# Kolkir/feature-point-cnn

Hardware: AMD Instinct MI355X
Metric: frames/sec (VGA 640x480) SuperPoint fwd+NMS+descriptors (higher is better)
Workload: dtype f32

## Files before the change

### feature-point-cnn_amd/_lib.py

```python
import ctypes
import os
import subprocess

import torch

_DIR = os.path.dirname(os.path.abspath(__file__))
LIB_PATH = os.environ.get("FPC_LIB_PATH") or os.path.join(_DIR, "lib", "libfpc.so")
CSRC = os.path.join(_DIR, "csrc")

SYMBOLS = [
    "fpc_abi_version", "fpc_build_flags", "fpc_strerror", "fpc_last_hip_error", "fpc_default_config", "fpc_create",
    "fpc_destroy", "fpc_load_weights", "fpc_packed_size", "fpc_packed_device_ptr",
    "fpc_export_packed", "fpc_import_packed", "fpc_import_packed_device", "fpc_mark_weights_loaded", "fpc_set_stream", "fpc_upload_stream",
    "fpc_get_stream", "fpc_sync", "fpc_forward", "fpc_detect", "fpc_get_points", "fpc_results",
    "fpc_get_counts", "fpc_get_keypoints", "fpc_set_timing", "fpc_get_timings", "fpc_match", "fpc_first_within",
    "fpc_detect_u8", "fpc_u8_staging", "fpc_homography_adaptation", "fpc_detect_u8_resized",
    "fpc_sample_descriptors", "fpc_plan_hash", "fpc_broadcast_weights", "fpc_read_activation",
    "fpc_pack_layout_revision", "fpc_check_guards", "fpc_stream_report", "fpc_output_range",
    "fpc_match_frames", "fpc_first_within_frames",
    "fpc_default_ransac_params", "fpc_ransac_homography", "fpc_homography_frames",
    "fpc_bank_create", "fpc_bank_destroy", "fpc_bank_get", "fpc_bank_store", "fpc_bank_store_rows", "fpc_bank_clear",
    "fpc_match_bank", "fpc_homography_bank", "fpc_bank_create_ex", "fpc_bank_format",
    "fpc_match_frames_guided", "fpc_match_bank_guided",
    "fpc_cell_order", "fpc_match_frames_guided_cells", "fpc_match_bank_guided_cells",
    "fpc_bank_topk_reserve", "fpc_match_bank_topk", "fpc_homography_bank_topk",
    "fpc_ransac_fundamental", "fpc_fundamental_frames", "fpc_fundamental_bank",
    "fpc_match_frames_guided_epipolar", "fpc_match_bank_guided_epipolar",
    "fpc_match_frames_guided_epipolar_cells", "fpc_match_bank_guided_epipolar_cells",
    "fpc_default_pose_params", "fpc_pose_fundamental", "fpc_pose_frames", "fpc_pose_bank",
]

ABI_VERSION = 4
PACK_LAYOUT_REVISION = 4

PLAN_FLAGS = {
    "no_fused_blocks": 1 << 0, "no_winograd": 1 << 1, "no_winograd_detector": 1 << 2, "no_winograd_layer_in1": 1 << 3,
    "no_xcd_order": 1 << 4, "no_fused_stem_pool": 1 << 5, "split_heads": 1 << 6, "nms_in_line": 1 << 7,
    "no_persistent_grid": 1 << 8, "layer1_tile_8x16": 1 << 9, "winograd_gen1": 1 << 10, "no_latency_tiles": 1 << 11,
    "nms_one_workgroup": 1 << 12, "no_fused_softmax": 1 << 13, "winograd_gen2": 1 << 14, "guard_zones": 1 << 15, "detector_gen1": 1 << 16, "heads_in_line": 1 << 17, "w36_one_wave": 1 << 18, "convt_phases": 1 << 19, "stem_round3": 1 << 20, "conv_round1": 1 << 21,
}


class FpcConfig(ctypes.Structure):
    _fields_ = [("device", ctypes.c_int), ("height", ctypes.c_int), ("width", ctypes.c_int),
                ("max_batch", ctypes.c_int), ("cell", ctypes.c_int), ("nms_dist", ctypes.c_int),
                ("conf_thresh", ctypes.c_float), ("border_remove", ctypes.c_int),
                ("descriptor_enabled", ctypes.c_int), ("max_keypoints", ctypes.c_int),
                ("in_channels", ctypes.c_int), ("dtype", ctypes.c_int), ("arch", ctypes.c_int),
                ("num_streams", ctypes.c_int), ("plan_flags", ctypes.c_uint), ("nms_round_launches", ctypes.c_int),
                ("min_sub_batch", ctypes.c_int)]


class FpcTensor(ctypes.Structure):
    _fields_ = [("name", ctypes.c_char_p), ("data", ctypes.c_void_p), ("ndim", ctypes.c_int),
# ... 172 lines not shown
```

### feature-point-cnn_amd/csrc/fpc_api.hip

```cpp
#include <hip/hip_runtime.h>

#include <dlfcn.h>

#include <algorithm>
#include <cmath>
#include <cstdio>
#include <cstdlib>
#include <cstring>
#include <memory>
#include <mutex>
#include <chrono>
#include <string>
#include <vector>

#include "../../include/fpc.h"
#include "block_mfma.h"
#include "block_bf16.h"
#include "convt_bf16.h"
#include "block_x3.h"
#include "stem_bf16.h"
#include "wblock_mfma.h"
#include "wblock16_mfma.h"
#include "wblock36_mfma.h"
#include "wblock36p_mfma.h"
// ... 194 lines not shown
      WK_COUNT
};

struct WKindInfo {
  const char* name;
  const char* symbol;
  int gen;
  int KC, NBT, CMID, lds_bytes;
  int NCG;
  int TH;
  int TW;
  int threads;
  const void* fn;
  void (*launch)(const WBlockArgs&, dim3, hipStream_t);
  bool dust = false;
};

#define X(name, KC, NBT, CMID)                                                                            \
  static void launchw_##name(const WBlockArgs& a, dim3 grid, hipStream_t st) {                            \
    constexpr int lds = WBlockCfg<KC, NBT, CMID>::LDS_BYTES;                                              \
    hipLaunchKernelGGL((wblock_mfma_kernel<KC, NBT, CMID>), grid, dim3(512), lds, st, a);                 \
  }
FPC_WBLOCK_KINDS(X)
#undef X
#define X(name, NCG, TH)                                                                                  \
  static void launchw_##name(const WBlockArgs& a, dim3 grid, hipStream_t st) {                            \
    constexpr int lds = W16Cfg<NCG, TH>::LDS_BYTES;                                                       \
    hipLaunchKernelGGL((wblock16_kernel<NCG, TH>), grid, dim3(512), lds, st, a);                          \
  }
FPC_W16_KINDS(X)
// ... 28 lines not shown
#undef X

static const WKindInfo g_wkinds[WK_COUNT] = {
#define X(name, KC, NBT, CMID)                                                                            \
  {#name, "wblock_mfma_kernel<" #KC ", " #NBT ", " #CMID ">", 1, KC, NBT, CMID,                           \
   WBlockCfg<KC, NBT, CMID>::LDS_BYTES, 0, 8, 16, 512, (const void*)wblock_mfma_kernel<KC, NBT, CMID>, launchw_##name},
    FPC_WBLOCK_KINDS(X)
#undef X
#define X(name, NCG, TH)                                                                                  \
  {#name, "wblock16_kernel<" #NCG ", " #TH ">", 2, 16, NCG / 2, NCG * 16,                                  \
   W16Cfg<NCG, TH>::LDS_BYTES, NCG, TH, 16, 512, (const void*)wblock16_kernel<NCG, TH>, launchw_##name},
    FPC_W16_KINDS(X)
#undef X
#define X(name, NB, TYT, TXT)                                                                             \
  {#name, "wblock36_kernel<" #NB ", " #TYT ", " #TXT ">", 3, 16, 2 * NB, 64 * NB,                          \
   W36Cfg<NB, TYT, TXT>::LDS_BYTES, 4 * NB, 4 * TYT, 4 * TXT, 256, (const void*)wblock36_kernel<NB, TYT, TXT>, launchw_##name},
    FPC_W36_KINDS(X)
#undef X
#define X(name, TYT, TXT)                                                                                 \
  {#name, "wblock36_dust_kernel<" #TYT ", " #TXT ">", 3, 16, 2, 64,                                        \
   W36Cfg<1, TYT, TXT, true>::LDS_BYTES, 4, 4 * TYT, 4 * TXT, 256, (const void*)wblock36_dust_kernel<TYT, TXT>, launchw_##name, true},
    FPC_W36D_KINDS(X)
#undef X
#define X(name, TYT, TXT)                                                                                 \
  {#name, "wblock36p_kernel<" #TYT ", " #TXT ", 3>", 3, 16, 2, 64,                                            \
   W36PCfg<TYT, TXT>::LDS_BYTES, 4, 4 * TYT, 4 * TXT, 512, (const void*)wblock36p_kernel<TYT, TXT>, launchw_##name},
    FPC_W36P_KINDS(X)
#undef X
#define X(name, TYT, TXT)                                                                                 \
  {#name, "wblock36p_dust_kernel<" #TYT ", " #TXT ", 3>", 3, 16, 2, 64,                                    \
   W36PCfg<TYT, TXT, true>::LDS_BYTES, 4, 4 * TYT, 4 * TXT, 512, (const void*)wblock36p_dust_kernel<TYT, TXT>, launchw_##name, true},
    FPC_W36PD_KINDS(X)
#undef X
};

static size_t w1_floats(const WKindInfo& k, int nchunk) {
  if (k.gen == 3) return (size_t)k.NCG * ((size_t)nchunk * 36 + (k.NCG == 8 ? W36Cfg<2, 4, 4>::WPAD : W36Cfg<1, 4, 4>::WPAD)) * 256;
  return (size_t)k.NCG * ((size_t)nchunk * 16 + W16Cfg<8>::WPAD) * 256;
}
static double wkind_mfma_flops(const WKindInfo& k, int tiles, int nchunk, int k8_1x1) {
  const double px = (double)k.TH * k.TW, n = k.NBT * 32.0;
  if (k.gen == 3) return 2.0 * tiles * n * (36.0 * (px / 16) * nchunk * k.KC + px * k8_1x1 * 8.0);
  return 2.0 * tiles * n * (16.0 * (px / 4) * nchunk * k.KC + px * k8_1x1 * 8.0);
}
static bool w36_fits(int , int H, int W, int cs_in, int cs_out) {
  return (unsigned long long)H * W * (unsigned long long)std::max(cs_in, cs_out) * sizeof(float) < (unsigned long long)W36_MARKER;
// ... 109 lines not shown
  int pH = 0, pW = 0, pC = 0;
  std::string prefix;
  int cin = 0, cout = 0;
  int grid_y = 1, grid_z = 1;
  double flops_per_frame = 0;
  double mfma_flops_per_frame = 0;
  bool fused_softmax_capable = false;
  double bytes_per_frame = 0;
  bool descriptor_branch = false;
};

struct Timing {
  hipEvent_t start, stop;
  int op;
  int frames;
};

}

using namespace fpc;

struct fpc_ctx {
  fpc_config cfg{};
  int H = 0, W = 0, B = 0, Hc = 0, Wc = 0;
  bool vgg = false;
  int D = 128;
  std::vector<float*> vbuf;
  size_t vconv0_off = 0;
  bool bf16 = false;
  bool split = false;
// ... 26 lines not shown
  bool logits_valid = false;
  bool nms_one_workgroup = false;
  int nms_g = 0;
  bool fuse_stem_pool = true;
  bool conv_lean = true;
  bool stem_lean = true;
  bool stem2 = false;
  bool layer1_t816 = false;
#ifdef FPC_DIAG
  unsigned long long* diag_stamps = nullptr;
  int diag_n = 0;
#endif
  bool winograd_in1 = true;
  bool winograd_det = true;
  int w36_cus = 0;
  bool w36_paired = true;
  bool winograd_det_gen3 = true;
  bool winograd = true;
  bool latency_tiles = true;
  int winograd_gen = 3;
  bool fuse_blocks = true;
  bool weights_loaded = false;
  bool plan_error = false;

  char* slab = nullptr;
  size_t slab_bytes = 0;
  bool guard_zones = false;
  std::vector<std::pair<size_t, size_t>> guards;
  float *stem_out, *x0, *h4, *x1, *x2, *h8, *x3, *cat, *dh, *dproj, *d0, *lg;
  float *h16, *y16a, *y16b, *lo_h, *lo0, *desc_map, *desc_in_nhwc;
// ... 1295 lines not shown
  c->stem2 = c->stem_lean && !c->bf16 && !c->split && !c->vgg && (c->fuse_stem_pool || c->cin == 1) && H2 % 2 == 0 && W2 % STEM_T == 0;
  return FPC_OK;
}

static uint64_t plan_hash(const fpc_ctx* c) {
  uint64_t h = 1469598103934665603ull;
  auto mix = [&](uint64_t v) {
    for (int i = 0; i < 8; ++i) {
      h ^= (v >> (8 * i)) & 0xff;
      h *= 1099511628211ull;
    }
  };
  mix(FPC_ABI_VERSION); mix(FPC_PACK_LAYOUT_REVISION); mix((uint64_t)c->cfg.dtype); mix((uint64_t)c->cfg.arch); mix((uint64_t)c->cin);
  mix((uint64_t)(c->cfg.descriptor_enabled != 0)); mix(c->blob_floats); mix(c->stem_w_off); mix(c->stem_b_off);
  mix(c->vconv0_off);
  for (size_t i = 0; i < c->ops.size(); ++i) {
    const Op& op = c->ops[i];
    mix((uint64_t)op.type); mix((uint64_t)op.kind); mix((uint64_t)op.bkind); mix((uint64_t)op.wkind); mix((uint64_t)op.fkind);
    mix((uint64_t)(op.phase + 1)); mix((uint64_t)op.n0);
    for (char ch : op.prefix) mix((uint64_t)(unsigned char)ch);
    const fpc_ctx::ConvW& cw = c->convw[i];
    for (int z = 0; z < 4; ++z) mix(cw.w_off[z]);
    mix(cw.b_off); mix(cw.b2_off);
  }
  return h;
}

static void fill_blob_header(const fpc_ctx* c, uint32_t* h) {
  memset(h, 0, BLOB_HEADER_FLOATS * sizeof(uint32_t));
  const uint64_t ph = plan_hash(c);
// ... 500 lines not shown
struct Sub {
  int f0, n;
  bool small = false;
  bool fuse_softmax = false;
  hipStream_t st;
  hipStream_t side = nullptr;
  hipEvent_t ev_enc = nullptr, ev_det = nullptr;
};

struct LaunchTimer {
  fpc_ctx* c;
  int op;
  hipStream_t st;
  int frames;
  hipEvent_t s{}, e{};
  LaunchTimer(fpc_ctx* c_, int op_, hipStream_t st_, int frames_) : c(c_), op(op_), st(st_), frames(frames_) {
    if (c->timing) {
      s = next_event(c);
      e = next_event(c);
      hipEventRecord(s, st);
    }
  }
  ~LaunchTimer() {
    if (c->timing) {
      hipEventRecord(e, st);
      c->timings.push_back({s, e, op, frames});
    }
  }
};

static int op_index(const fpc_ctx* c, OpType t) {
  for (size_t i = 0; i < c->ops.size(); ++i)
    if (c->ops[i].type == t) return (int)i;
  return -1;
}

static void run_network(fpc_ctx* c, const float* frames, const Sub& sb0, int which, hipStream_t st) {
  Sub sb = sb0;
  sb.st = st;
  const int H = c->H, W = c->W, n = sb.n, f0 = sb.f0;
  for (size_t i = 0; i < c->ops.size(); ++i) {
// ... 88 lines not shown
            a.stamps = c->diag_stamps;
            c->diag_n = a.tiles_x * a.tiles_y * n;
          }
#endif
        a.total = a.tiles_x * a.tiles_y * n;
        a.xcd_order = c->xcd_order ? 1 : 0;
        {
          const unsigned long long xb = (unsigned long long)(f0 + n) * a.H * a.W * a.csx * sizeof(float);
          a.x_bytes = xb > 0xfffffff0ull ? 0xfffffff0u : (unsigned)xb;
        }
        int grid = (c->persist_min_tiles > 0 && a.total >= c->persist_min_tiles * c->num_cus) ? c->num_cus : a.total;
        if (g_wkinds[op.wkind].gen == 3) {
          const int fpl = w36_frames_per_launch(a.H, a.W, a.csx, a.cso);
          const float* x0 = a.x;
          float* o0 = a.out;
          for (int g0 = 0; g0 < n; g0 += fpl) {
            const int gn = std::min(fpl, n - g0);
            a.frame0 = 0;
            a.x = x0 + (size_t)(f0 + g0) * a.H * a.W * a.csx;
            a.out = o0 + (size_t)(f0 + g0) * a.H * a.W * a.cso;
            a.total = a.tiles_x * a.tiles_y * gn;
            a.x_bytes = (unsigned)((unsigned long long)gn * a.H * a.W * a.csx * sizeof(float));
            const int cus_cap = c->w36_cus > 0 ? std::min(c->num_cus, c->w36_cus) : c->num_cus;
            const int cus8 = std::max(1, cus_cap / 8 / std::max(1, op.grid_y)), per_xcd = (a.total + 7) / 8;
            const int rounds = (per_xcd + cus8 - 1) / cus8;
            const int grid3 = 8 * std::min(cus8, (per_xcd + rounds - 1) / rounds);
            g_wkinds[op.wkind].launch(a, dim3(std::min(a.total, grid3), op.grid_y), sb.st);
          }
          break;
        }
        g_wkinds[op.wkind].launch(a, dim3(std::min(a.total, grid), op.grid_y), sb.st);
        break;
      }
      case OP_BLOCK: {
        LaunchTimer t(c, (int)i, sb.st, n);
        BlockArgs a = op.bargs;
        a.frame0 = f0;
#ifdef FPC_DIAG
        a.stamps = nullptr;
        if (const char* e = getenv("FPC_STAMP_OP"))
          if (op.name.find(e) != std::string::npos) {
            if (!c->diag_stamps) hipHostMalloc((void**)&c->diag_stamps, (size_t)65536 * 8 * sizeof(unsigned long long));
            memset(c->diag_stamps, 0, (size_t)65536 * 8 * sizeof(unsigned long long));
// ... 373 lines not shown
  const auto create_t0 = std::chrono::steady_clock::now();
  std::unique_lock<std::mutex> queue_lock(qmap::state().mu);
  const int probe_rounds0 = qmap::state().dev[cfg->device].rounds;
  c->stream = qmap::acquire(cfg->device, c.get(), SLOT_MAIN, true, qprobe, true);
  if (!c->stream) { qmap::release_owner(c.get()); g_hip_err = "hipStreamCreateWithFlags"; return FPC_E_HIP; }
  c->own_stream = true;
  {
    int nsub = cfg->num_streams > 0 ? std::min(8, cfg->num_streams) : (c->split ? 3 : 2);
    const unsigned pf = cfg->plan_flags;
    c->fuse_blocks = !(pf & FPC_PLAN_NO_FUSED_BLOCKS);
    c->guard_zones = (pf & FPC_PLAN_GUARD_ZONES) != 0;
    if (const char* e = getenv("FPC_GUARD_ZONES")) c->guard_zones = atoi(e) != 0;
    c->winograd_det_gen3 = !(pf & FPC_PLAN_DETECTOR_GEN1);
    c->w36_paired = !(pf & FPC_PLAN_W36_ONE_WAVE);
    if (const char* e = getenv("FPC_W36_PAIRED")) c->w36_paired = atoi(e) != 0;
    if (const char* e = getenv("FPC_W36_CUS")) c->w36_cus = std::max(0, atoi(e));
    if (const char* e = getenv("FPC_WINOGRAD_DET_GEN")) c->winograd_det_gen3 = atoi(e) >= 3;
    c->winograd = !(pf & FPC_PLAN_NO_WINOGRAD);
    c->winograd_det = !(pf & FPC_PLAN_NO_WINOGRAD_DETECTOR);
    c->winograd_in1 = !(pf & FPC_PLAN_NO_WINOGRAD_LAYER_IN1);
    c->xcd_order = !(pf & FPC_PLAN_NO_XCD_ORDER);
    c->fuse_stem_pool = !(pf & FPC_PLAN_NO_FUSED_STEM_POOL);
    c->stem_lean = !(pf & FPC_PLAN_STEM_ROUND3);
    c->conv_lean = !(pf & FPC_PLAN_CONV_ROUND1);
    if (const char* e = getenv("FPC_CONV_LEAN")) c->conv_lean = atoi(e) != 0;
    if (const char* e = getenv("FPC_STEM_LEAN")) c->stem_lean = atoi(e) != 0;
    c->split_heads = (pf & FPC_PLAN_SPLIT_HEADS) != 0;
    if (pf & FPC_PLAN_NO_PERSISTENT_GRID) c->persist_min_tiles = 0;
    c->layer1_t816 = (pf & FPC_PLAN_LAYER1_TILE_8x16) != 0;
    c->winograd_gen = (pf & FPC_PLAN_WINOGRAD_GEN1) ? 1 : (pf & FPC_PLAN_WINOGRAD_GEN2) ? 2 : 3;
// ... 1466 lines not shown
          case OP_CONV: k = op->lean ? lean_kind(op->kind)->symbol : g_kinds[op->kind].symbol; break;
          case OP_BLOCK: k = g_bkinds[op->bkind].symbol; break;
          case OP_WBLOCK: k = g_wkinds[op->wkind].symbol; break;
          case OP_BF16: k = g_fkinds[op->fkind].symbol; break;
          case OP_SOFTMAX: k = "softmax_d2s_kernel"; break;
          case OP_NMS: k = c->nms_one_workgroup ? "nms_rounds_kernel+nms_sort_kernel" : "nms_rounds_kernel+nms_finish_kernel+nms_chunk_sort_kernel+nms_merge_kernel"; break;
          case OP_DESC: k = "descriptor16_kernel"; break;
          case OP_VCONV0: k = "vgg_conv0_kernel"; break;
          case OP_POOL2: k = "maxpool2_kernel"; break;
          case OP_L2NORM: k = "l2norm256_kernel"; break;
        }
      kernels[i] = k;
    }
    if (ms) ms[i] = v;
    if (flops) flops[i] = op ? op->flops_per_frame * t.frames : 0.0;
    if (mfma_flops) mfma_flops[i] = op ? op->mfma_flops_per_frame * t.frames : 0.0;
    if (bytes) bytes[i] = op ? op->bytes_per_frame * t.frames : 0.0;
  }
  return n;
}

}
```

### feature-point-cnn_amd/csrc/wblock36_mfma.h

```cpp
#pragma once
#include <type_traits>
#include <utility>

#include "wblock16_mfma.h"

namespace fpc {

template <int... I, class F>
__device__ __forceinline__ void fpc_static_for_impl(std::integer_sequence<int, I...>, F&& f) {
  (f(std::integral_constant<int, I>{}), ...);
}
template <int N, class F>
__device__ __forceinline__ void fpc_static_for(F&& f) {
  fpc_static_for_impl(std::make_integer_sequence<int, N>{}, f);
}

struct W36Dust {
  static constexpr int W2ROW = 0, W2COL = 64, WPCOL = 144, B1 = 400, B2 = 401, UIN64 = 404, UIN = 448, UOUT = 448 + 4 * 36 * 16;
  static constexpr int floats(int nchunk) { return UOUT + nchunk * 36 * 16; }
};

template <int NB_, int TYT_, int TXT_, bool DUST_ = false>
struct W36Cfg {
  static constexpr int NB = NB_, TYT = TYT_, TXT = TXT_;
// ... 188 lines not shown
  auto t_burst = [&]() {
#pragma unroll
    for (int jj = 0; jj < 3; ++jj) bt6(tp[0][jj], tp[1][jj], tp[2][jj], tp[3][jj], tp[4][jj], tp[5][jj]);
#pragma unroll
    for (int ii = 0; ii < 3; ++ii)
#pragma unroll
      for (int jj = 0; jj < 3; ++jj) {
        const f32x2 ra = tp[2 * ii][jj], rb = tp[2 * ii + 1][jj];
        tp[2 * ii][jj] = __builtin_shufflevector(ra, rb, 0, 2);
        tp[2 * ii + 1][jj] = __builtin_shufflevector(ra, rb, 1, 3);
      }
#pragma unroll
    for (int ii = 0; ii < 3; ++ii) bt6(tp[2 * ii][0], tp[2 * ii + 1][0], tp[2 * ii][1], tp[2 * ii + 1][1], tp[2 * ii][2], tp[2 * ii + 1][2]);
  };
  auto t_write = [&](int wr, int i, int j) { lds[wr + (i * 6 + j) * 256] = tp[2 * (i >> 1) + (j & 1)][j >> 1][i & 1]; };
  auto transform_all = [&](int hoff, int voff) {
#pragma unroll
    for (int i = 0; i < 6; ++i)
#pragma unroll
      for (int j = 0; j < 6; ++j) t_read(trd + hoff, i, j);
    t_burst();
#pragma unroll
    for (int i = 0; i < 6; ++i)
#pragma unroll
      for (int j = 0; j < 6; ++j) t_write(twr + voff, i, j);
  };

  const int aoff4 = (lane & 15) * 4 + ((lane >> 4) ^ (2 * ((lane & 15) >> 3)));
  const unsigned gstride = ((unsigned)nchunk * 36u + (unsigned)C::WPAD) * 1024u;
  const __amdgpu_buffer_rsrc_t wrsrc = __builtin_amdgcn_make_buffer_rsrc(const_cast<float4*>(w1h), 0, (int)(4u * (unsigned)NB * gstride), 0x00020000);
  const unsigned wlane = (unsigned)(wave * NB) * gstride + lane16;
  const int gs_s = __builtin_amdgcn_readfirstlane((int)gstride);
  struct BF { f32x4 v[2][NB]; };
  auto ldb = [&](int s) {
    BF r;
// ... 13 lines not shown
  if constexpr (DUST) {
    d_va = wave * 64 + lane;
    d_ua = wave * 64 + 16 * ((lane & 3) ^ (2 * (lane >> 5)));
    for (int i = tid; i < 448 / 4; i += NT) lds4[C::D_HEAD / 4 + i] = reinterpret_cast<const f32x4*>(a.dust)[i];
    for (int i = tid; i < 2304 / 4; i += NT) lds4[C::D_UIN / 4 + i] = reinterpret_cast<const f32x4*>(a.dust + W36Dust::UIN)[i];
  }

  TilePos pos_cur = tile_pos(wg_first);
  int base_cur = halo_base(pos_cur);
  halo_tile(pos_cur);
  load_halo64(base_cur);
  load_halo(base_cur, C::OFF_H0);
  load_halo(base_cur + 64, C::OFF_H1);
  asm volatile("s_waitcnt vmcnt(%0)" ::"n"(HIT) : "memory");
  FPC_LDS_BARRIER();
  transform_all(C::OFF_H0, C::OFF_V0);
  FPC_LDS_BARRIER();

  constexpr int C4 = N / 4, EIT = HPX * C4 / NT, PPI = NT / C4;
  constexpr int CPR = TW / PPI;
  const __amdgpu_buffer_rsrc_t orsrc = __builtin_amdgcn_make_buffer_rsrc(a.out + blockIdx.y * N, 0, W36_MARKER, 0x00020000);

  const int g2s = __builtin_amdgcn_readfirstlane(((a.k8_h + a.k8_x) / 2 + C::WPAD2) * 64);
  const __amdgpu_buffer_rsrc_t w2rsrc = __builtin_amdgcn_make_buffer_rsrc(const_cast<float4*>(a.w2), 0, a.conv_only ? 0 : 4 * NB * g2s * 16, 0x00020000);
  const unsigned w2lane = (unsigned)(wave * NB * g2s) * 16u + lane16;

  const int wg_stamp = wg_first + 2 * wg_step < wg_end ? wg_first + 2 * wg_step : wg_first;
  for (int wg = wg_first; wg < wg_end; wg += wg_step) {
    const int b = pos_cur.b, ty = pos_cur.ty, tx = pos_cur.tx;
    const TilePos pos_next = tile_pos(wg + wg_step);
// ... 16 lines not shown
    if constexpr (DUST) {
      float zf = 0.f;
      asm volatile("" : "+v"(zf));
#pragma unroll
      for (int i = 0; i < 9; ++i) dacc[i] = zf;
    }

    auto chunk_body = [&](auto PAR, const int c) {
      constexpr int par = decltype(PAR)::value;
      constexpr int VB_OFF = par ? C::OFF_V1 : C::OFF_V0, VN_OFF = par ? C::OFF_V0 : C::OFF_V1;
      constexpr int HS_OFF = par ? C::OFF_H1 : C::OFF_H0;
      constexpr int HN_OFF = par ? C::OFF_H0 : C::OFF_H1;
      const int c3 = c + 2;
      const bool nxt = c3 >= nchunk;
      const int l_base = (nxt ? base_next : base_cur) + (nxt ? c3 - nchunk : c3) * 64;
      int ao = aoff4 + VB_OFF / 4, trd_c = trd + HN_OFF, twr_c = twr + VN_OFF;
      asm volatile("" : "+v"(ao), "+v"(trd_c), "+v"(twr_c));
      [[maybe_unused]] int dva = d_va + VB_OFF / 4;
      [[maybe_unused]] f32x4 dv[3];
      if constexpr (DUST) asm volatile("" : "+v"(dva));
      constexpr int AQ = 2;
      f32x4 ac[2][AQ];
#pragma unroll
      for (int q = 0; q < AQ; ++q) ac[0][q] = lds4[ao + q * 64];
#ifdef FPC_DIAG_STEPS
      unsigned long long tq[11] = {0, 0, 0, 0, 0, 0, 0, 0, 0, 0, 0};
#define FPC_TQ(i) asm volatile("s_memtime %0" : "=s"(tq[i]));
#else
#define FPC_TQ(i)
#endif
      fpc_static_for<STEPS>([&](auto S) __attribute__((always_inline)) {
        constexpr int s = decltype(S)::value;
        if constexpr (s % 2 == 0) { FPC_TQ(s / 2) }
        bq[(s + RING - 1) % RING] = ldb(c * STEPS + s + RING - 1);
        if (s + 1 < STEPS) {
#pragma unroll
          for (int q = 0; q < AQ; ++q) ac[(s + 1) & 1][q] = lds4[ao + ((s + 1) * AQ + q) * 64];
        }
        constexpr int SPS = 36 / STEPS;
#pragma unroll
        for (int u = 0; u < SPS; ++u) {
          const int slot = s * SPS + u;
          if (slot == 1) {
            if (c3 == nchunk) halo_tile(pos_next);
            load_halo(l_base, HS_OFF);
          } else if (slot >= 2 && slot < 14) {
#pragma unroll
            for (int k = 0; k < 3; ++k) { const int e = (slot - 2) * 3 + k; t_read(trd_c, e / 6, e % 6); }
          } else if (slot == 14) {
            t_burst();
          } else if (slot >= 15 && slot < 33) {
#pragma unroll
            for (int k = 0; k < 2; ++k) { const int e = (slot - 15) * 2 + k; t_write(twr_c, e / 6, e % 6); }
          }
          if constexpr (DUST) {
            auto dread = [&](int i0) {
#pragma unroll
              for (int k = 0; k < 3; ++k) dv[k] = lds4[dva + (i0 + k) * 256];
            };
            auto dfma = [&](int i0) {
#pragma unroll
              for (int k = 0; k < 3; ++k)
#pragma unroll
// ... 28 lines not shown
        }
        __builtin_amdgcn_sched_barrier(0);
      });
      FPC_TQ(9)
      asm volatile("s_waitcnt vmcnt(%0)" ::"n"(2 * NB * (RING - 1)) : "memory");
      FPC_LDS_BARRIER();
      FPC_TQ(10)
#ifdef FPC_DIAG_STEPS
      if (a.stamps && wg == wg_stamp && c == 2 && (threadIdx.x & 63) == 0) {
        asm volatile("s_waitcnt lgkmcnt(0)" ::: "memory");
        unsigned long long* q = a.stamps + 1024 * 8 + ((size_t)blockIdx.x * 4 + (threadIdx.x >> 6)) * 16;
        for (int i = 0; i < 11; ++i) q[i] = tq[i];
      }
#endif
    };
    __builtin_amdgcn_s_waitcnt(0x0F70);
    {
      int c = 0;
      do {
        chunk_body(std::integral_constant<int, 0>{}, c);
        chunk_body(std::integral_constant<int, 1>{}, c + 1);
        c += 2;
      } while (c < nchunk);
    }
    if (wg == wg_stamp) { FPC_STAMP(1) }
    asm volatile("s_nop 15\n\ts_nop 7" ::: "memory");

    if constexpr (DUST) {
      int tid_d = tid;
      asm volatile("" : "+v"(tid_d));
// ... 430 lines not shown
```

### feature-point-cnn_amd/csrc/wblock36p_mfma.h

```cpp
#pragma once
#include "wblock36_mfma.h"

namespace fpc {

template <int TYT_, int TXT_, bool DUST_ = false>
struct W36PCfg {
  static constexpr int TYT = TYT_, TXT = TXT_;
  static constexpr bool DUST = DUST_;
  static_assert(TYT * TXT == 16 && (TYT == 4 || TYT == 2), "16 Winograd tiles per workgroup tile: 4 x 4 or 2 x 8");
  static constexpr int NT = 512, NTH = 256, NPOS = 36, KC = 16, N = 64;
  static constexpr int TH = 4 * TYT, TW = 4 * TXT, HH = TH + 2, HW = TW + 2, NHALO = HH * HW;
  static constexpr int HROW = 20;
  static constexpr int HIT = (NHALO * 5 + NTH - 1) / NTH;
  static constexpr int HALO_FLOATS = HIT * NTH * 4;
  static constexpr int V_FLOATS = NPOS * 16 * 16;
  static constexpr int OFF_V0 = 0, OFF_H1 = V_FLOATS, OFF_H0 = OFF_H1 + HALO_FLOATS, OFF_V1 = OFF_H0 + HALO_FLOATS;
  static constexpr int RH = N + 8;
  static constexpr int PX = TH * TW;
  static constexpr int T_FLOATS = PX * RH;
  static constexpr int BASE_FLOATS = (OFF_V1 + V_FLOATS) > (OFF_H0 + T_FLOATS) ? (OFF_V1 + V_FLOATS) : (OFF_H0 + T_FLOATS);
  static constexpr int HIT64 = (NHALO + NTH - 1) / NTH;
  static constexpr int D_HEAD = BASE_FLOATS, D_COL = D_HEAD + 64, D_UIN = D_HEAD + 448, D_V64 = D_UIN + 2304, D_M64 = D_V64 + 576, D_H64 = D_M64 + 576;
  static constexpr int LDS_FLOATS = DUST ? D_H64 + HIT64 * NTH * 4 : BASE_FLOATS;
  static constexpr int LDS_BYTES = LDS_FLOATS * 4;
// ... 144 lines not shown
  auto t_burst = [&]() {
#pragma unroll
    for (int jj = 0; jj < 3; ++jj) bt6(tp[0][jj], tp[1][jj], tp[2][jj], tp[3][jj], tp[4][jj], tp[5][jj]);
#pragma unroll
    for (int ii = 0; ii < 3; ++ii)
#pragma unroll
      for (int jj = 0; jj < 3; ++jj) {
        const f32x2 ra = tp[2 * ii][jj], rb = tp[2 * ii + 1][jj];
        tp[2 * ii][jj] = __builtin_shufflevector(ra, rb, 0, 2);
        tp[2 * ii + 1][jj] = __builtin_shufflevector(ra, rb, 1, 3);
      }
#pragma unroll
    for (int ii = 0; ii < 3; ++ii) bt6(tp[2 * ii][0], tp[2 * ii + 1][0], tp[2 * ii][1], tp[2 * ii + 1][1], tp[2 * ii][2], tp[2 * ii + 1][2]);
  };
  auto t_write = [&](int wr, int i, int j) { lds[wr + (i * 6 + j) * 256] = tp[2 * (i >> 1) + (j & 1)][j >> 1][i & 1]; };

  const int aoff4 = (lane & 15) * 4 + ((lane >> 4) ^ (2 * ((lane & 15) >> 3))) + hs * 18 * 64;
  const unsigned gstride = ((unsigned)nchunk * 36u + (unsigned)C::WPAD) * 1024u;
  const __amdgpu_buffer_rsrc_t wrsrc = __builtin_amdgcn_make_buffer_rsrc(const_cast<float4*>(w1h), 0, (int)(4u * gstride), 0x00020000);
  const unsigned wlane = (unsigned)grp * gstride + (unsigned)hs * (18u * 1024u) + lane16;
  struct BF { f32x4 v[2]; };
  auto ldb = [&](int cc, int s) {
    BF r;
#pragma unroll
    for (int q = 0; q < 2; ++q)
      r.v[q] = __builtin_bit_cast(f32x4, __builtin_amdgcn_raw_buffer_load_b128(wrsrc, (int)wlane, cc * (36 * 1024) + (2 * s + q) * 1024, 0));
    return r;
  };

  [[maybe_unused]] int d_va = 0, d_ua = 0;
// ... 7 lines not shown
    for (int i = tid; i < 448 / 4; i += C::NT) lds4[C::D_HEAD / 4 + i] = reinterpret_cast<const f32x4*>(a.dust)[i];
    for (int i = tid; i < 2304 / 4; i += C::NT) lds4[C::D_UIN / 4 + i] = reinterpret_cast<const f32x4*>(a.dust + W36Dust::UIN)[i];
  }

  TilePos pos_cur = tile_pos(wg_first);
  int base_cur = halo_base(pos_cur);
  if (hs == 1) {
    halo_tile(pos_cur);
    load_halo64(base_cur);
    load_halo(base_cur, C::OFF_H0);
    load_halo(base_cur + 64, C::OFF_H1);
    asm volatile("s_waitcnt vmcnt(%0)" ::"n"(HIT) : "memory");
  }
  FPC_LDS_BARRIER();
  if (hs == 0) {
#pragma unroll
    for (int i = 0; i < 6; ++i)
#pragma unroll
      for (int j = 0; j < 6; ++j) t_read(trd + C::OFF_H0, i, j);
    t_burst();
#pragma unroll
    for (int i = 0; i < 6; ++i)
#pragma unroll
      for (int j = 0; j < 6; ++j) t_write(twr + C::OFF_V0, i, j);
  }
  FPC_LDS_BARRIER();

  constexpr int C4 = N / 4, EIT = PX * C4 / C::NT, PPI = C::NT / C4;
  constexpr int RPI = PPI / TW > 0 ? PPI / TW : 1;
  const __amdgpu_buffer_rsrc_t orsrc = __builtin_amdgcn_make_buffer_rsrc(a.out + blockIdx.y * N, 0, W36_MARKER, 0x00020000);
  const int g2s = __builtin_amdgcn_readfirstlane(((a.k8_h + a.k8_x) / 2 + C::WPAD2) * 64);
  const __amdgpu_buffer_rsrc_t w2rsrc = __builtin_amdgcn_make_buffer_rsrc(const_cast<float4*>(a.w2), 0, a.conv_only ? 0 : 4 * g2s * 16, 0x00020000);
  const unsigned w2lane = (unsigned)(grp * g2s) * 16u + lane16;

// ... 17 lines not shown
#pragma unroll
      for (int i = 0; i < 9; ++i) dacc[i] = zf;
    }
    BF bq[RING];
#pragma unroll
    for (int i = 0; i < RING - 1; ++i) bq[i] = ldb(0, i);

    auto chunk_body = [&](auto ROLE, auto PAR, const int c) {
      constexpr int role = decltype(ROLE)::value, par = decltype(PAR)::value;
      constexpr int VB_OFF = par ? C::OFF_V1 : C::OFF_V0, VN_OFF = par ? C::OFF_V0 : C::OFF_V1;
      constexpr int HS_OFF = par ? C::OFF_H1 : C::OFF_H0;
      constexpr int HN_OFF = par ? C::OFF_H0 : C::OFF_H1;
      const int c3 = c + 2;
      const bool nxt = c3 >= nchunk;
      const int l_base = (nxt ? base_next : base_cur) + (nxt ? c3 - nchunk : c3) * 64;
      int ao = aoff4 + VB_OFF / 4, trd_c = trd + HN_OFF, twr_c = twr + VN_OFF;
      asm volatile("" : "+v"(ao), "+v"(trd_c), "+v"(twr_c));
      [[maybe_unused]] int dva = d_va + VB_OFF / 4;
      [[maybe_unused]] f32x4 dv[3];
      if constexpr (DUST) asm volatile("" : "+v"(dva));
      f32x4 ac[2][2];
#pragma unroll
      for (int q = 0; q < 2; ++q) ac[0][q] = lds4[ao + q * 64];
      fpc_static_for<STEPS>([&](auto S) __attribute__((always_inline)) {
        constexpr int s = decltype(S)::value;
        {
          constexpr int t = s + RING - 1;
          if constexpr (t < STEPS) bq[t % RING] = ldb(c, t);
          else bq[t % RING] = ldb(c + 1, t - STEPS);
        }
        if (s + 1 < STEPS) {
#pragma unroll
// ... 23 lines not shown
#pragma unroll
                for (int k = 0; k < 3; ++k)
                  du[(i0 / 3 % 2) * 3 + k] = __builtin_bit_cast(f32x4, __builtin_amdgcn_raw_buffer_load_b128(drsrc, d_ua + (i0 + k) * 256, c * (36 * 16 * 4), 0));
              };
              if (slot == 3) dload(0);
              else if (slot == 11) dread(0);
              else if (slot == 13) { dfma(0); dload(3); }
              else if (slot == 21) dread(3);
              else if (slot == 23) { dfma(3); dload(6); }
              else if (slot == 31) dread(6);
              else if (slot == 33) dfma(6);
            }
          } else {
            if (slot >= 2 && slot < 14) {
#pragma unroll
              for (int k = 0; k < 3; ++k) { const int e = (slot - 2) * 3 + k; t_read(trd_c, e / 6, e % 6); }
            } else if (slot == 14) {
              t_burst();
            } else if (slot >= 15 && slot < 33) {
#pragma unroll
              for (int k = 0; k < 2; ++k) { const int e = (slot - 15) * 2 + k; t_write(twr_c, e / 6, e % 6); }
            }
          }
        }
        __builtin_amdgcn_sched_barrier(0);
        fpc_mfma_step<false, false>(acc[2 * s], acc[2 * s + 1], ac[s & 1][0], ac[s & 1][1], bq[s % RING].v[0], bq[s % RING].v[1]);
        __builtin_amdgcn_sched_barrier(0);
      });
      asm volatile("s_waitcnt vmcnt(%0)" ::"n"(2 * (STEPS - 1)) : "memory");
      FPC_LDS_BARRIER();
    };
    __builtin_amdgcn_s_waitcnt(0x0F70);
    if (hs == 0) {
      int c = 0;
      do {
        chunk_body(std::integral_constant<int, 0>{}, std::integral_constant<int, 0>{}, c);
        chunk_body(std::integral_constant<int, 0>{}, std::integral_constant<int, 1>{}, c + 1);
        c += 2;
      } while (c < nchunk);
    } else {
      int c = 0;
      do {
        chunk_body(std::integral_constant<int, 1>{}, std::integral_constant<int, 0>{}, c);
        chunk_body(std::integral_constant<int, 1>{}, std::integral_constant<int, 1>{}, c + 1);
        c += 2;
      } while (c < nchunk);
    }
    if (wg == wg_stamp) { FPC_STAMP(1) }
    asm volatile("s_nop 15\n\ts_nop 7" ::: "memory");

    int tid_t = tid;
    asm volatile("" : "+v"(tid_t));
    const int lane_t = tid_t & 63, n16 = lane_t & 15, kq = lane_t >> 4;
    const bool proj = a.k8_x > 0;
    if constexpr (DUST) {
      if (a.dust_in) {
        if (tid_t < 16) {
          const int rd = C::D_H64 + ((4 * (tid_t / TXT)) * HW + 4 * (tid_t % TXT)) * 4;
#pragma unroll
          for (int i = 0; i < 6; ++i)
#pragma unroll
            for (int j = 0; j < 6; ++j) tp[i][j >> 1][j & 1] = lds[rd + (i * HW + j) * 4];
          t_burst();
          const int mrow = ((tid_t & 7) >> 1) * 4 + (tid_t >> 3) * 2 + (tid_t & 1);
#pragma unroll
          for (int i = 0; i < 6; ++i)
#pragma unroll
            for (int j = 0; j < 6; ++j) lds[C::D_V64 + (i * 6 + j) * 16 + mrow] = tp[2 * (i >> 1) + (j & 1)][j >> 1][i & 1];
        }
        FPC_LDS_BARRIER();
        {
          const int va = C::D_V64 + hs * 18 * 16 + (lane_t & 15), ub = C::D_UIN + grp * 576 + hs * 18 * 16 + (lane_t & 15);
          float av[18], bv[18];
#pragma unroll
          for (int p = 0; p < 18; ++p) {
            av[p] = lds[va + p * 16];
            bv[p] = lds[ub + p * 16];
// ... 216 lines not shown
            cb[(u + 3) & 3] = ldb2(s_first + g + u + 3);
            fpc_static_for<4>([&](auto B_) __attribute__((always_inline)) {
              constexpr int blk = decltype(B_)::value;
              if (blk + 1 < 4) {
#pragma unroll
                for (int q = 0; q < 2; ++q) af[(blk + 1) & 1][q] = lds4[ar + (g + u) * 4 + ((blk + 1) * 2 + q) * 16 * (RH / 4)];
              } else {
#pragma unroll
                for (int q = 0; q < 2; ++q) af[(blk + 1) & 1][q] = lds4[ar + (g + u + 1) * 4 + q * 16 * (RH / 4)];
              }
              __builtin_amdgcn_sched_barrier(0);
              fpc_mfma_step<false, false>(acc2[2 * blk], acc2[2 * blk + 1], af[blk & 1][0], af[blk & 1][1], cb[u], cb[u]);
              __builtin_amdgcn_sched_barrier(0);
            });
          }
        }
      };
      if (proj) {
        constexpr int XIT = PX * 16 / C::NT;
        f32x4 xst[XIT];
        auto load_x = [&](int pass) {
          const int kx4 = min(16, a.k8_x * 2 - pass * 16);
          const int px0 = tid_t >> 4;
          const int xp = (((px0 / TW) * a.W + px0 % TW) * a.csx + ((tid_t & 15) < kx4 ? pass * 64 + (tid_t & 15) * 4 : 0)) * 4;
#pragma unroll
          for (int i = 0; i < XIT; ++i) {
            const int so = xbase + i * RPI * a.W * a.csx * 4;
            xst[i] = __builtin_bit_cast(f32x4, __builtin_amdgcn_raw_buffer_load_b128(xrsrc, xp + so, 0, 0));
          }
        };
// ... 116 lines not shown
```

### feature-point-cnn_amd/csrc/wblock_mfma.h

```cpp
#pragma once
#include "block_mfma.h"

namespace fpc {

struct WBlockArgs {
  const float* x;
  int csx, nchunk;
  int H, W;
  const float4* w1;
  const float* b1;
  const float4* w2;
  const float* b2;
  int k8_h, k8_x;
  float* out;
  int cso, tiles_x, tiles_y, frame0;
  int total;
  int xcd_order;
  int ysplit_floats;
  unsigned x_bytes;
  int conv_only;
  const float* dust;
  int dust_in;
#ifdef FPC_DIAG
  unsigned long long* stamps;
#endif
};

template <int KC, int NBT, int CMID_>
struct WBlockCfg {
  static constexpr int TH = 8, TW = 16, NT = 512;
  static constexpr int HW = TW + 2, HH = TH + 2;
  static constexpr int ROW4 = KC / 4 + 1;
  static constexpr int CMID = CMID_;
  static constexpr int ROWH4 = CMID / 4 + 1;
  static constexpr int HALO_BYTES = HH * HW * ROW4 * 16;
  static constexpr int V_BYTES = 16 * 32 * ROW4 * 16;
  static constexpr int M_BYTES = 16 * 32 * 36 * 4;
// ... 408 lines not shown
```

### include/fpc.h

```cpp
#ifndef FPC_H
#define FPC_H

#include <stddef.h>
#include <stdint.h>

#ifdef __cplusplus
extern "C" {
#endif

#define FPC_ABI_VERSION 4
#define FPC_PACK_LAYOUT_REVISION 4

enum {
  FPC_OK = 0,
  FPC_E_INVALID = -1,
  FPC_E_NO_DEVICE = -2,
  FPC_E_HIP = -3,
  FPC_E_NO_WEIGHTS = -4,
  FPC_E_MISSING_KEY = -5,
  FPC_E_CAPACITY = -6,
  FPC_E_NOT_CONVERGED = -7,
  FPC_E_RANGE = -8,
  FPC_E_NONFINITE = -9
};
// ... 30 lines not shown
  FPC_PLAN_NO_FUSED_STEM_POOL = 1 << 5,
  FPC_PLAN_SPLIT_HEADS = 1 << 6,
  FPC_PLAN_NMS_IN_LINE = 1 << 7,
  FPC_PLAN_NO_PERSISTENT_GRID = 1 << 8,
  FPC_PLAN_LAYER1_TILE_8x16 = 1 << 9,
  FPC_PLAN_WINOGRAD_GEN1 = 1 << 10,
  FPC_PLAN_NO_LATENCY_TILES = 1 << 11,
  FPC_PLAN_NMS_ONE_WORKGROUP = 1 << 12,
  FPC_PLAN_NO_FUSED_SOFTMAX = 1 << 13,
  FPC_PLAN_WINOGRAD_GEN2 = 1 << 14,
  FPC_PLAN_HEADS_IN_LINE = 1 << 17,
  FPC_PLAN_DETECTOR_GEN1 = 1 << 16,
  FPC_PLAN_W36_ONE_WAVE = 1 << 18,
  FPC_PLAN_STEM_ROUND3 = 1 << 20,
  FPC_PLAN_CONV_ROUND1 = 1 << 21,
  FPC_PLAN_CONVT_PHASES = 1 << 19,
  FPC_PLAN_GUARD_ZONES = 1 << 15
};

typedef struct fpc_tensor {
  const char* name;
  const float* data;
  int ndim;
  int64_t shape[4];
} fpc_tensor;

typedef struct fpc_device_results {
  const int32_t* count;
  const int32_t* n_candidates;
  const int32_t* xy;
// ... 199 lines not shown
```

Measured before the change: 12090.

## Stack frames vertically in Winograd F(4,3) kernels to avoid partial edge tiles

When the frame height is a multiple of 4 but not of 16, the Winograd block kernels now treat a group of frames as one tall image, so 16-row tiles span frame boundaries instead of each frame ending in a partly empty tile. Rows that touch a frame boundary are redirected to zero-padding in LDS, using a magic-number modulo to find the per-frame row. This cuts wasted tile work at frame edges in exchange for extra per-tile index arithmetic and added complexity. Timing accounting scales MFMA flops by the number of tiles actually walked, and a plan flag and env var can turn the behaviour off.

Result: no change. 12180 (median of 6 runs) (+0.8%).

```diff
diff --git a/feature-point-cnn_amd/_lib.py b/feature-point-cnn_amd/_lib.py
--- a/feature-point-cnn_amd/_lib.py
+++ b/feature-point-cnn_amd/_lib.py
@@ -38,6 +38,7 @@
     "no_xcd_order": 1 << 4, "no_fused_stem_pool": 1 << 5, "split_heads": 1 << 6, "nms_in_line": 1 << 7,
     "no_persistent_grid": 1 << 8, "layer1_tile_8x16": 1 << 9, "winograd_gen1": 1 << 10, "no_latency_tiles": 1 << 11,
     "nms_one_workgroup": 1 << 12, "no_fused_softmax": 1 << 13, "winograd_gen2": 1 << 14, "guard_zones": 1 << 15, "detector_gen1": 1 << 16, "heads_in_line": 1 << 17, "w36_one_wave": 1 << 18, "convt_phases": 1 << 19, "stem_round3": 1 << 20, "conv_round1": 1 << 21,
+    "w36_no_stack": 1 << 22,
 }
 
 
diff --git a/feature-point-cnn_amd/csrc/fpc_api.hip b/feature-point-cnn_amd/csrc/fpc_api.hip
--- a/feature-point-cnn_amd/csrc/fpc_api.hip
+++ b/feature-point-cnn_amd/csrc/fpc_api.hip
@@ -232,6 +232,7 @@
   const void* fn;
   void (*launch)(const WBlockArgs&, dim3, hipStream_t);
   bool dust = false;
+  bool stack = false;
 };
 
 #define X(name, KC, NBT, CMID)                                                                            \
@@ -290,7 +291,8 @@
 #undef X
 #define X(name, NB, TYT, TXT)                                                                             \
   {#name, "wblock36_kernel<" #NB ", " #TYT ", " #TXT ">", 3, 16, 2 * NB, 64 * NB,                          \
-   W36Cfg<NB, TYT, TXT>::LDS_BYTES, 4 * NB, 4 * TYT, 4 * TXT, 256, (const void*)wblock36_kernel<NB, TYT, TXT>, launchw_##name},
+   W36Cfg<NB, TYT, TXT>::LDS_BYTES, 4 * NB, 4 * TYT, 4 * TXT, 256, (const void*)wblock36_kernel<NB, TYT, TXT>, launchw_##name, \
+   false, NB == 2 && TYT == 4},
     FPC_W36_KINDS(X)
 #undef X
 #define X(name, TYT, TXT)                                                                                 \
@@ -300,12 +302,14 @@
 #undef X
 #define X(name, TYT, TXT)                                                                                 \
   {#name, "wblock36p_kernel<" #TYT ", " #TXT ", 3>", 3, 16, 2, 64,                                            \
-   W36PCfg<TYT, TXT>::LDS_BYTES, 4, 4 * TYT, 4 * TXT, 512, (const void*)wblock36p_kernel<TYT, TXT>, launchw_##name},
+   W36PCfg<TYT, TXT>::LDS_BYTES, 4, 4 * TYT, 4 * TXT, 512, (const void*)wblock36p_kernel<TYT, TXT>, launchw_##name, false, \
+   TYT == 4},
     FPC_W36P_KINDS(X)
 #undef X
 #define X(name, TYT, TXT)                                                                                 \
   {#name, "wblock36p_dust_kernel<" #TYT ", " #TXT ", 3>", 3, 16, 2, 64,                                    \
-   W36PCfg<TYT, TXT, true>::LDS_BYTES, 4, 4 * TYT, 4 * TXT, 512, (const void*)wblock36p_dust_kernel<TYT, TXT>, launchw_##name, true},
+   W36PCfg<TYT, TXT, true>::LDS_BYTES, 4, 4 * TYT, 4 * TXT, 512, (const void*)wblock36p_dust_kernel<TYT, TXT>, launchw_##name, true, \
+   TYT == 4},
     FPC_W36PD_KINDS(X)
 #undef X
 };
@@ -445,6 +449,7 @@
   hipEvent_t start, stop;
   int op;
   int frames;
+  double mfma_scale = 1.0;
 };
 
 }
@@ -501,6 +506,7 @@
   bool winograd_in1 = true;
   bool winograd_det = true;
   int w36_cus = 0;
+  bool w36_stack = true;
   bool w36_paired = true;
   bool winograd_det_gen3 = true;
   bool winograd = true;
@@ -1826,6 +1832,7 @@
   mix(FPC_ABI_VERSION); mix(FPC_PACK_LAYOUT_REVISION); mix((uint64_t)c->cfg.dtype); mix((uint64_t)c->cfg.arch); mix((uint64_t)c->cin);
   mix((uint64_t)(c->cfg.descriptor_enabled != 0)); mix(c->blob_floats); mix(c->stem_w_off); mix(c->stem_b_off);
   mix(c->vconv0_off);
+  if (!c->w36_stack) mix(0x5733364e4f53544bull);
   for (size_t i = 0; i < c->ops.size(); ++i) {
     const Op& op = c->ops[i];
     mix((uint64_t)op.type); mix((uint64_t)op.kind); mix((uint64_t)op.bkind); mix((uint64_t)op.wkind); mix((uint64_t)op.fkind);
@@ -2356,6 +2363,7 @@
   hipStream_t st;
   int frames;
   hipEvent_t s{}, e{};
+  double mfma_scale = 1.0;
   LaunchTimer(fpc_ctx* c_, int op_, hipStream_t st_, int frames_) : c(c_), op(op_), st(st_), frames(frames_) {
     if (c->timing) {
       s = next_event(c);
@@ -2366,7 +2374,7 @@
   ~LaunchTimer() {
     if (c->timing) {
       hipEventRecord(e, st);
-      c->timings.push_back({s, e, op, frames});
+      c->timings.push_back({s, e, op, frames, mfma_scale});
     }
   }
 };
@@ -2485,19 +2493,29 @@
           const int fpl = w36_frames_per_launch(a.H, a.W, a.csx, a.cso);
           const float* x0 = a.x;
           float* o0 = a.out;
+          const int H1 = a.H, tiles_y1 = a.tiles_y;
+          const bool stackable = c->w36_stack && g_wkinds[op.wkind].stack && g_wkinds[op.wkind].TH == 16 && H1 % 4 == 0 && H1 % 16 != 0;
+          long long walked = 0;
           for (int g0 = 0; g0 < n; g0 += fpl) {
             const int gn = std::min(fpl, n - g0);
+            const bool stacked = stackable && gn >= 2 && (long long)gn * H1 + 16 < 65536;
             a.frame0 = 0;
-            a.x = x0 + (size_t)(f0 + g0) * a.H * a.W * a.csx;
-            a.out = o0 + (size_t)(f0 + g0) * a.H * a.W * a.cso;
-            a.total = a.tiles_x * a.tiles_y * gn;
-            a.x_bytes = (unsigned)((unsigned long long)gn * a.H * a.W * a.csx * sizeof(float));
+            a.x = x0 + (size_t)(f0 + g0) * H1 * a.W * a.csx;
+            a.out = o0 + (size_t)(f0 + g0) * H1 * a.W * a.cso;
+            a.H = stacked ? gn * H1 : H1;
+            a.tiles_y = stacked ? (gn * H1 + 15) / 16 : tiles_y1;
+            a.stack_h = stacked ? H1 : 0;
+            a.stack_magic = stacked ? (unsigned)(0x100000000ull / (unsigned)H1) + 1u : 0u;
+            a.total = stacked ? a.tiles_x * a.tiles_y : a.tiles_x * a.tiles_y * gn;
+            a.x_bytes = (unsigned)((unsigned long long)gn * H1 * a.W * a.csx * sizeof(float));
             const int cus_cap = c->w36_cus > 0 ? std::min(c->num_cus, c->w36_cus) : c->num_cus;
             const int cus8 = std::max(1, cus_cap / 8 / std::max(1, op.grid_y)), per_xcd = (a.total + 7) / 8;
             const int rounds = (per_xcd + cus8 - 1) / cus8;
             const int grid3 = 8 * std::min(cus8, (per_xcd + rounds - 1) / rounds);
             g_wkinds[op.wkind].launch(a, dim3(std::min(a.total, grid3), op.grid_y), sb.st);
+            walked += a.total;
           }
+          t.mfma_scale = (double)walked / ((double)a.tiles_x * tiles_y1 * n);
           break;
         }
         g_wkinds[op.wkind].launch(a, dim3(std::min(a.total, grid), op.grid_y), sb.st);
@@ -2901,6 +2919,8 @@
     c->winograd_det_gen3 = !(pf & FPC_PLAN_DETECTOR_GEN1);
     c->w36_paired = !(pf & FPC_PLAN_W36_ONE_WAVE);
     if (const char* e = getenv("FPC_W36_PAIRED")) c->w36_paired = atoi(e) != 0;
+    c->w36_stack = !(pf & FPC_PLAN_W36_NO_STACK);
+    if (const char* e = getenv("FPC_W36_STACK")) c->w36_stack = atoi(e) != 0;
     if (const char* e = getenv("FPC_W36_CUS")) c->w36_cus = std::max(0, atoi(e));
     if (const char* e = getenv("FPC_WINOGRAD_DET_GEN")) c->winograd_det_gen3 = atoi(e) >= 3;
     c->winograd = !(pf & FPC_PLAN_NO_WINOGRAD);
@@ -4397,7 +4417,7 @@
     }
     if (ms) ms[i] = v;
     if (flops) flops[i] = op ? op->flops_per_frame * t.frames : 0.0;
-    if (mfma_flops) mfma_flops[i] = op ? op->mfma_flops_per_frame * t.frames : 0.0;
+    if (mfma_flops) mfma_flops[i] = op ? op->mfma_flops_per_frame * t.frames * t.mfma_scale : 0.0;
     if (bytes) bytes[i] = op ? op->bytes_per_frame * t.frames : 0.0;
   }
   return n;
diff --git a/feature-point-cnn_amd/csrc/wblock36_mfma.h b/feature-point-cnn_amd/csrc/wblock36_mfma.h
--- a/feature-point-cnn_amd/csrc/wblock36_mfma.h
+++ b/feature-point-cnn_amd/csrc/wblock36_mfma.h
@@ -226,11 +226,25 @@
     for (int ii = 0; ii < 3; ++ii) bt6(tp[2 * ii][0], tp[2 * ii + 1][0], tp[2 * ii][1], tp[2 * ii + 1][1], tp[2 * ii][2], tp[2 * ii + 1][2]);
   };
   auto t_write = [&](int wr, int i, int j) { lds[wr + (i * 6 + j) * 256] = tp[2 * (i >> 1) + (j & 1)][j >> 1][i & 1]; };
+  constexpr bool STACK = NB == 2 && TYT == 4 && !DUST;
+  [[maybe_unused]] int zr0 = 0, zr5 = 0;
+  auto stack_rows = [&](const TilePos& q) {
+    if constexpr (STACK) {
+      const unsigned sh = (unsigned)a.stack_h;
+      const unsigned y = (unsigned)(q.ty * TH + 4 * wave);
+      const unsigned m = y - __umulhi(y, a.stack_magic) * sh;
+      int tl = tid;
+      asm volatile("" : "+v"(tl));
+      const int zo = 16 - (tl & 15);
+      zr0 = ((sh != 0) & (m == 0)) ? zo : 0;
+      zr5 = ((sh != 0) & (m + 4 == sh)) ? zo : 0;
+    }
+  };
   auto transform_all = [&](int hoff, int voff) {
 #pragma unroll
     for (int i = 0; i < 6; ++i)
 #pragma unroll
-      for (int j = 0; j < 6; ++j) t_read(trd + hoff, i, j);
+      for (int j = 0; j < 6; ++j) t_read(trd + hoff + (i == 0 ? zr0 : i == 5 ? zr5 : 0), i, j);
     t_burst();
 #pragma unroll
     for (int i = 0; i < 6; ++i)
@@ -274,6 +288,7 @@
   load_halo(base_cur + 64, C::OFF_H1);
   asm volatile("s_waitcnt vmcnt(%0)" ::"n"(HIT) : "memory");
   FPC_LDS_BARRIER();
+  stack_rows(pos_cur);
   transform_all(C::OFF_H0, C::OFF_V0);
   FPC_LDS_BARRIER();
 
@@ -320,8 +335,12 @@
       const int c3 = c + 2;
       const bool nxt = c3 >= nchunk;
       const int l_base = (nxt ? base_next : base_cur) + (nxt ? c3 - nchunk : c3) * 64;
+      if constexpr (STACK && par == 1) {
+        if (c + 1 == nchunk) stack_rows(pos_next);
+      }
       int ao = aoff4 + VB_OFF / 4, trd_c = trd + HN_OFF, twr_c = twr + VN_OFF;
       asm volatile("" : "+v"(ao), "+v"(trd_c), "+v"(twr_c));
+      [[maybe_unused]] const int trd_0 = trd_c + zr0, trd_5 = trd_c + zr5;
       [[maybe_unused]] int dva = d_va + VB_OFF / 4;
       [[maybe_unused]] f32x4 dv[3];
       if constexpr (DUST) asm volatile("" : "+v"(dva));
@@ -352,7 +371,7 @@
             load_halo(l_base, HS_OFF);
           } else if (slot >= 2 && slot < 14) {
 #pragma unroll
-            for (int k = 0; k < 3; ++k) { const int e = (slot - 2) * 3 + k; t_read(trd_c, e / 6, e % 6); }
+            for (int k = 0; k < 3; ++k) { const int e = (slot - 2) * 3 + k; t_read(!STACK ? trd_c : e / 6 == 0 ? trd_0 : e / 6 == 5 ? trd_5 : trd_c, e / 6, e % 6); }
           } else if (slot == 14) {
             t_burst();
           } else if (slot >= 15 && slot < 33) {
@@ -411,6 +430,7 @@
       }
 #endif
     };
+    stack_rows(pos_cur);
     __builtin_amdgcn_s_waitcnt(0x0F70);
     {
       int c = 0;
diff --git a/feature-point-cnn_amd/csrc/wblock36p_mfma.h b/feature-point-cnn_amd/csrc/wblock36p_mfma.h
--- a/feature-point-cnn_amd/csrc/wblock36p_mfma.h
+++ b/feature-point-cnn_amd/csrc/wblock36p_mfma.h
@@ -182,6 +182,20 @@
     for (int ii = 0; ii < 3; ++ii) bt6(tp[2 * ii][0], tp[2 * ii + 1][0], tp[2 * ii][1], tp[2 * ii + 1][1], tp[2 * ii][2], tp[2 * ii + 1][2]);
   };
   auto t_write = [&](int wr, int i, int j) { lds[wr + (i * 6 + j) * 256] = tp[2 * (i >> 1) + (j & 1)][j >> 1][i & 1]; };
+  constexpr bool STACK = TYT == 4;
+  [[maybe_unused]] int zr0 = 0, zr5 = 0;
+  auto stack_rows = [&](const TilePos& q) {
+    if constexpr (STACK) {
+      const unsigned sh = (unsigned)a.stack_h;
+      const unsigned y = (unsigned)(q.ty * TH + 4 * grp);
+      const unsigned m = y - __umulhi(y, a.stack_magic) * sh;
+      int tl = tid;
+      asm volatile("" : "+v"(tl));
+      const int zo = 16 - (tl & 15);
+      zr0 = ((sh != 0) & (m == 0)) ? zo : 0;
+      zr5 = ((sh != 0) & (m + 4 == sh)) ? zo : 0;
+    }
+  };
 
   const int aoff4 = (lane & 15) * 4 + ((lane >> 4) ^ (2 * ((lane & 15) >> 3))) + hs * 18 * 64;
   const unsigned gstride = ((unsigned)nchunk * 36u + (unsigned)C::WPAD) * 1024u;
@@ -219,10 +233,11 @@
   }
   FPC_LDS_BARRIER();
   if (hs == 0) {
+    stack_rows(pos_cur);
 #pragma unroll
     for (int i = 0; i < 6; ++i)
 #pragma unroll
-      for (int j = 0; j < 6; ++j) t_read(trd + C::OFF_H0, i, j);
+      for (int j = 0; j < 6; ++j) t_read(trd + C::OFF_H0 + (i == 0 ? zr0 : i == 5 ? zr5 : 0), i, j);
     t_burst();
 #pragma unroll
     for (int i = 0; i < 6; ++i)
@@ -270,8 +285,12 @@
       const int c3 = c + 2;
       const bool nxt = c3 >= nchunk;
       const int l_base = (nxt ? base_next : base_cur) + (nxt ? c3 - nchunk : c3) * 64;
+      if constexpr (STACK && role == 0 && par == 1) {
+        if (c + 1 == nchunk) stack_rows(pos_next);
+      }
       int ao = aoff4 + VB_OFF / 4, trd_c = trd + HN_OFF, twr_c = twr + VN_OFF;
       asm volatile("" : "+v"(ao), "+v"(trd_c), "+v"(twr_c));
+      [[maybe_unused]] const int trd_0 = trd_c + zr0, trd_5 = trd_c + zr5;
       [[maybe_unused]] int dva = d_va + VB_OFF / 4;
       [[maybe_unused]] f32x4 dv[3];
       if constexpr (DUST) asm volatile("" : "+v"(dva));
@@ -325,7 +344,7 @@
           } else {
             if (slot >= 2 && slot < 14) {
 #pragma unroll
-              for (int k = 0; k < 3; ++k) { const int e = (slot - 2) * 3 + k; t_read(trd_c, e / 6, e % 6); }
+              for (int k = 0; k < 3; ++k) { const int e = (slot - 2) * 3 + k; t_read(!STACK ? trd_c : e / 6 == 0 ? trd_0 : e / 6 == 5 ? trd_5 : trd_c, e / 6, e % 6); }
             } else if (slot == 14) {
               t_burst();
             } else if (slot >= 15 && slot < 33) {
@@ -343,6 +362,7 @@
     };
     __builtin_amdgcn_s_waitcnt(0x0F70);
     if (hs == 0) {
+      stack_rows(pos_cur);
       int c = 0;
       do {
         chunk_body(std::integral_constant<int, 0>{}, std::integral_constant<int, 0>{}, c);
@@ -368,10 +388,18 @@
       if (a.dust_in) {
         if (tid_t < 16) {
           const int rd = C::D_H64 + ((4 * (tid_t / TXT)) * HW + 4 * (tid_t % TXT)) * 4;
+          int rd0 = rd, rd5 = rd;
+          if constexpr (STACK) {
+            const unsigned sh = (unsigned)a.stack_h;
+            const unsigned y = (unsigned)(ty * TH + 4 * (tid_t / TXT));
+            const unsigned m = y - __umulhi(y, a.stack_magic) * sh;
+            rd0 += (sh != 0) & (m == 0);
+            rd5 += (sh != 0) & (m + 4 == sh);
+          }
 #pragma unroll
           for (int i = 0; i < 6; ++i)
 #pragma unroll
-            for (int j = 0; j < 6; ++j) tp[i][j >> 1][j & 1] = lds[rd + (i * HW + j) * 4];
+            for (int j = 0; j < 6; ++j) tp[i][j >> 1][j & 1] = lds[(i == 0 ? rd0 : i == 5 ? rd5 : rd) + (i * HW + j) * 4];
           t_burst();
           const int mrow = ((tid_t & 7) >> 1) * 4 + (tid_t >> 3) * 2 + (tid_t & 1);
 #pragma unroll
@@ -618,6 +646,7 @@
               __builtin_amdgcn_sched_barrier(0);
             });
           }
+          asm volatile("s_nop 0" ::: "memory");
         }
       };
       if (proj) {
diff --git a/feature-point-cnn_amd/csrc/wblock_mfma.h b/feature-point-cnn_amd/csrc/wblock_mfma.h
--- a/feature-point-cnn_amd/csrc/wblock_mfma.h
+++ b/feature-point-cnn_amd/csrc/wblock_mfma.h
@@ -21,6 +21,8 @@
   int conv_only;
   const float* dust;
   int dust_in;
+  int stack_h;
+  unsigned stack_magic;
 #ifdef FPC_DIAG
   unsigned long long* stamps;
 #endif
diff --git a/include/fpc.h b/include/fpc.h
--- a/include/fpc.h
+++ b/include/fpc.h
@@ -68,6 +68,7 @@
   FPC_PLAN_W36_ONE_WAVE = 1 << 18,
   FPC_PLAN_STEM_ROUND3 = 1 << 20,
   FPC_PLAN_CONV_ROUND1 = 1 << 21,
+  FPC_PLAN_W36_NO_STACK = 1 << 22,
   FPC_PLAN_CONVT_PHASES = 1 << 19,
   FPC_PLAN_GUARD_ZONES = 1 << 15
 };
```
